# haidog-yaqub/EzAudio

Hardware: NVIDIA H100
Metric: audio-seconds generated per wall-second (EzAudio-XL, 50-step DDIM, 10 s) (higher is better)
Workload: dtype bf16

## Files before the change

### ezaudio_b200/csrc/common.cuh

```cuda
#pragma once
#include <cuda.h>
#include <cuda_bf16.h>
#include <cuda_runtime.h>
#include <stdint.h>

#include "wgmma.cuh"

namespace ezb {

__device__ __forceinline__ uint32_t smem_u32(const void* p) { return (uint32_t)__cvta_generic_to_shared(p); }

__device__ __forceinline__ bool elect_one() {
  uint32_t pred;
  asm volatile(
      "{\n\t.reg .pred p;\n\telect.sync _|p, 0xffffffff;\n\tselp.u32 %0, 1, 0, p;\n\t}\n"
      : "=r"(pred));
  return pred != 0;
}

__device__ __forceinline__ void pdl_wait() { asm volatile("griddepcontrol.wait;" ::: "memory"); }
__device__ __forceinline__ void pdl_launch() { asm volatile("griddepcontrol.launch_dependents;" ::: "memory"); }

__device__ __forceinline__ void mbar_init(uint64_t* bar, uint32_t count) {
  asm volatile("mbarrier.init.shared::cta.b64 [%0], %1;" ::"r"(smem_u32(bar)), "r"(count));
}
__device__ __forceinline__ void fence_mbar_init() { asm volatile("fence.mbarrier_init.release.cluster;" ::: "memory"); }
__device__ __forceinline__ void mbar_expect_tx(uint64_t* bar, uint32_t bytes) {
  asm volatile("mbarrier.arrive.expect_tx.shared::cta.b64 _, [%0], %1;" ::"r"(smem_u32(bar)), "r"(bytes) : "memory");
}
__device__ __forceinline__ void mbar_arrive(uint64_t* bar) {
  asm volatile("mbarrier.arrive.shared::cta.b64 _, [%0];" ::"r"(smem_u32(bar)) : "memory");
}
__device__ __forceinline__ void mbar_wait(uint64_t* bar, uint32_t parity) {
  asm volatile(
      "{\n\t.reg .pred P1;\n\t"
      "WAIT_LOOP:\n\t"
      "mbarrier.try_wait.parity.shared::cta.b64 P1, [%0], %1, 0x989680;\n\t"
      "@P1 bra DONE;\n\t"
      "bra WAIT_LOOP;\n\t"
      "DONE:\n\t}\n" ::"r"(smem_u32(bar)),
      "r"(parity)
      : "memory");
}

__device__ __forceinline__ void fence_proxy_async_smem() { asm volatile("fence.proxy.async.shared::cta;" ::: "memory"); }
__device__ __forceinline__ void named_bar_sync(int id, int nthreads) {
  asm volatile("bar.sync %0, %1;" ::"r"(id), "r"(nthreads) : "memory");
}

__device__ __forceinline__ void tma_prefetch_desc(const CUtensorMap* m) {
  asm volatile("prefetch.tensormap [%0];" ::"l"(reinterpret_cast<uint64_t>(m)) : "memory");
}
__device__ __forceinline__ void tma_load_2d(void* dst, const CUtensorMap* m, uint64_t* bar, int c0, int c1) {
  asm volatile(
      "cp.async.bulk.tensor.2d.shared::cluster.global.mbarrier::complete_tx::bytes [%0], [%1, {%3, %4}], [%2];" ::"r"(
          smem_u32(dst)),
      "l"(reinterpret_cast<uint64_t>(m)), "r"(smem_u32(bar)), "r"(c0), "r"(c1)
      : "memory");
}
__device__ __forceinline__ void tma_load_3d(void* dst, const CUtensorMap* m, uint64_t* bar, int c0, int c1, int c2) {
  asm volatile(
      "cp.async.bulk.tensor.3d.shared::cluster.global.mbarrier::complete_tx::bytes [%0], [%1, {%3, %4, %5}], [%2];" ::"r"(
          smem_u32(dst)),
      "l"(reinterpret_cast<uint64_t>(m)), "r"(smem_u32(bar)), "r"(c0), "r"(c1), "r"(c2)
      : "memory");
}

__device__ __forceinline__ void tma_load_4d(void* dst, const CUtensorMap* m, uint64_t* bar, int c0, int c1, int c2, int c3) {
  asm volatile(
      "cp.async.bulk.tensor.4d.shared::cluster.global.mbarrier::complete_tx::bytes [%0], [%1, {%3, %4, %5, %6}], [%2];" ::"r"(
          smem_u32(dst)),
      "l"(reinterpret_cast<uint64_t>(m)), "r"(smem_u32(bar)), "r"(c0), "r"(c1), "r"(c2), "r"(c3)
      : "memory");
}
__device__ __forceinline__ void tma_store_2d(const CUtensorMap* m, const void* src, int c0, int c1) {
  asm volatile("cp.async.bulk.tensor.2d.global.shared::cta.bulk_group [%0, {%2, %3}], [%1];" ::"l"(reinterpret_cast<uint64_t>(m)),
               "r"(smem_u32(src)), "r"(c0), "r"(c1)
               : "memory");
}
__device__ __forceinline__ void bulk_commit_group() { asm volatile("cp.async.bulk.commit_group;" ::: "memory"); }
template <int N>
__device__ __forceinline__ void bulk_wait_group_read() { asm volatile("cp.async.bulk.wait_group.read %0;" ::"n"(N) : "memory"); }
template <int N>
__device__ __forceinline__ void bulk_wait_group() { asm volatile("cp.async.bulk.wait_group %0;" ::"n"(N) : "memory"); }

__device__ __forceinline__ uint64_t wgmma_desc_sw128(uint32_t smem_addr) {
  uint64_t d = 0;
  d |= (uint64_t)((smem_addr & 0x3FFFF) >> 4);
  d |= (uint64_t)1 << 16;
  d |= (uint64_t)(1024 >> 4) << 32;
  d |= (uint64_t)1 << 62;
  return d;
}
__device__ __forceinline__ uint64_t wgmma_desc_sw32(uint32_t smem_addr) {
  uint64_t d = 0;
  d |= (uint64_t)((smem_addr & 0x3FFFF) >> 4);
  d |= (uint64_t)1 << 16;
  d |= (uint64_t)(256 >> 4) << 32;
  d |= (uint64_t)3 << 62;
  return d;
}
__device__ __forceinline__ void wgmma_fence() { asm volatile("wgmma.fence.sync.aligned;" ::: "memory"); }
__device__ __forceinline__ void wgmma_commit() { asm volatile("wgmma.commit_group.sync.aligned;" ::: "memory"); }
template <int N>
__device__ __forceinline__ void wgmma_wait() { asm volatile("wgmma.wait_group.sync.aligned %0;" ::"n"(N) : "memory"); }
template <int R>
__device__ __forceinline__ void wgmma_fence_regs(float (&d)[R]) {
#pragma unroll
  for (int i = 0; i < R; ++i) asm volatile("" : "+f"(d[i])::"memory");
}

__device__ __forceinline__ float gelu_erf(float x) { return 0.5f * x * (1.0f + erff(x * 0.70710678118654752440f)); }
__device__ __forceinline__ float silu(float x) { return x / (1.0f + expf(-x)); }
__device__ __forceinline__ uint32_t pack_bf16(float a, float b) {
  __nv_bfloat162 v = __floats2bfloat162_rn(a, b);
  return *reinterpret_cast<uint32_t*>(&v);
}
__device__ __forceinline__ float warp_sum(float v) {
#pragma unroll
  for (int o = 16; o > 0; o >>= 1) v += __shfl_xor_sync(0xffffffffu, v, o);
  return v;
}
__device__ __forceinline__ float warp_max(float v) {
#pragma unroll
  for (int o = 16; o > 0; o >>= 1) v = fmaxf(v, __shfl_xor_sync(0xffffffffu, v, o));
  return v;
}

}

namespace ezb {
__device__ __forceinline__ uint32_t cluster_ctarank() {
  uint32_t r;
  asm volatile("mov.u32 %0, %%cluster_ctarank;" : "=r"(r));
  return r;
}
__device__ __forceinline__ void cluster_sync_all() {
  asm volatile("barrier.cluster.arrive.release.aligned;" ::: "memory");
  asm volatile("barrier.cluster.wait.acquire.aligned;" ::: "memory");
}
__device__ __forceinline__ uint32_t mapa_u32(uint32_t local_addr, uint32_t rank) {
  uint32_t r;
  asm volatile("mapa.shared::cluster.u32 %0, %1, %2;" : "=r"(r) : "r"(local_addr), "r"(rank));
  return r;
}
__device__ __forceinline__ void mbar_arrive_cluster(uint32_t cluster_addr) {
  asm volatile("mbarrier.arrive.release.cluster.shared::cluster.b64 _, [%0];" ::"r"(cluster_addr) : "memory");
}
__device__ __forceinline__ void mbar_arrive_cluster_nofence(uint32_t cluster_addr) {
  asm volatile("mbarrier.arrive.shared::cluster.b64 _, [%0];" ::"r"(cluster_addr) : "memory");
}
__device__ __forceinline__ void mbar_inval(uint64_t* bar) {
  asm volatile("mbarrier.inval.shared::cta.b64 [%0];" ::"r"(smem_u32(bar)) : "memory");
}
__device__ __forceinline__ void tma_load_2d_mc(void* dst, const CUtensorMap* m, uint64_t* bar, int c0, int c1, uint16_t mask) {
  asm volatile(
      "cp.async.bulk.tensor.2d.shared::cluster.global.mbarrier::complete_tx::bytes.multicast::cluster [%0], [%1, {%3, %4}], [%2], %5;" ::"r"(
          smem_u32(dst)),
      "l"(reinterpret_cast<uint64_t>(m)), "r"(smem_u32(bar)), "r"(c0), "r"(c1), "h"(mask)
      : "memory");
}
}
```

### ezaudio_b200/csrc/gemm.cuh

```cuda
#pragma once
#include "common.cuh"

namespace ezb {

constexpr int GEMM_BM = 128;
constexpr int GEMM_BK = 64;
#ifdef EZB_GEMM_DEBUG
#define EZB_DBG(...) __VA_ARGS__
#else
#define EZB_DBG(...)
#endif
constexpr int GEMM_SMEM_BUDGET = 227 * 1024 - 2048;
constexpr int gemm_b_box(int bn) { return bn > 256 ? bn / 2 : bn; }

struct GemmShape {
  int M, N;
  int num_k_blocks;
  int num_m_tiles, num_n_tiles;
  int taps, center, dilation, cin_blocks, T, tiles_per_batch;
  int stride, pad;
  unsigned long long* dbg;
  const char* pf;
  unsigned int pf_bytes;
};
// ... 301 lines not shown
    const EpiLinearParams& e = ep.lin;
    const int nv = nvalid < 32 ? nvalid : 32;
    wait();
#pragma unroll 1
    for (int c = c_begin; c < c_end; c += 64) {
      const int col = n0 + c + 2 * lane;
      const bool col_ok = (c + 2 * lane < c_end) && col < N;
      __syncwarp();
#pragma unroll
      for (int hc = 0; hc < 2; ++hc) {
        uint32_t r[32];
        acc_ld<32>(ar, c + 32 * hc, lane, r);
#pragma unroll
        for (int g = 0; g < 16; ++g) stage_put(st, lane, 16 * hc + g, __uint_as_float(r[2 * g]), __uint_as_float(r[2 * g + 1]));
      }
      __syncwarp();
      if (!col_ok) continue;
      const float b0 = e.bias != nullptr ? e.bias[col] : 0.f, b1 = e.bias != nullptr ? e.bias[col + 1] : 0.f;
#pragma unroll 4
      for (int rr = 0; rr < nv; ++rr) {
        const int row = row0 + rr;
        const float s = ep.scale[row / ep.rows_per_batch];
        const float2 acc = stage_get(st, rr, lane);
        *reinterpret_cast<float2*>(e.out_f32 + (size_t)row * e.ld32 + col) = make_float2((acc.x + b0) * s, (acc.y + b1) * s);
      }
    }
  }
};

struct EpiGegluParams {
  const float* bias;
  __nv_bfloat16* out_bf16;
  int ld16;
  int split_stride;
  FoldIn fin;
};
__device__ __forceinline__ float rcp_approx(float x) {
  float r;
  asm("rcp.approx.ftz.f32 %0, %1;" : "=f"(r) : "f"(x));
  return r;
}
__device__ __forceinline__ float ex2_approx(float x) {
  float r;
  asm("ex2.approx.ftz.f32 %0, %1;" : "=f"(r) : "f"(x));
  return r;
}
__device__ __forceinline__ float geglu_fast(float h, float g) {
  const float z = g * 0.70710678118654752440f, az = fabsf(z);
  const float t = rcp_approx(fmaf(0.3275911f, az, 1.0f));
  float p = fmaf(1.061405429f, t, -1.453152027f);
  p = fmaf(p, t, 1.421413741f);
  p = fmaf(p, t, -0.284496736f);
  p = fmaf(p, t, 0.254829592f);
  const float e = ex2_approx(az * az * -1.4426950408889634f);
  const float erf_abs = fmaf(-p * t, e, 1.0f);
  const float erf_s = copysignf(erf_abs, z);
  return h * (0.5f * g) * (1.0f + erf_s);
}

template <int BN, bool FOLD = false>
struct EpiGeglu {
  using Params = EpiGegluParams;
  static constexpr int HALF = BN / 2;
  static constexpr int EPI_WARPS = BN == 256 ? 8 : 4;
  static constexpr bool WIDE_REGS = false;
  static constexpr int STAGE_FLOATS = 32 * 32;
  template <class Wait>
  static __device__ __forceinline__ void run(const Params& ep, float* st, const AccRows& ar, int row0, int nvalid, int n0, int N, int lane, int c_begin,
                                             int c_end, Wait wait) {
    constexpr bool fold = FOLD;
    float rstd = 1.f, nmr = 0.f;
    if (fold && lane < nvalid) fold_row_stats(ep.fin, row0 + lane, rstd, nmr);
    wait();
    const int f_begin = c_begin / 2, f_end = c_end / 2;
#pragma unroll 1
    for (int c = f_begin; c < f_end; c += 64) {
      if (n0 + c >= N) break;
      if (ep.split_stride > 0) {
        uint32_t h[32], g[32];
#pragma unroll 1
        for (int q4 = 0; q4 < 2; ++q4) {
          __syncwarp();
          acc_ld<32>(ar, c + q4 * 32, lane, h);
          acc_ld<32>(ar, HALF + c + q4 * 32, lane, g);
          if (lane < nvalid) {
            __nv_bfloat16* o = ep.out_bf16 + (size_t)(row0 + lane) * ep.ld16 + (n0 / 2 + c + q4 * 32);
#pragma unroll
            for (int j = 0; j < 32; j += 2) {
              const float o0 = (__uint_as_float(h[j]) + ep.bias[n0 + c + q4 * 32 + j]) * gelu_erf(__uint_as_float(g[j]) + ep.bias[n0 + HALF + c + q4 * 32 + j]);
              const float o1 = (__uint_as_float(h[j + 1]) + ep.bias[n0 + c + q4 * 32 + j + 1]) * gelu_erf(__uint_as_float(g[j + 1]) + ep.bias[n0 + HALF + c + q4 * 32 + j + 1]);
              store_bf16x2(o + j, ep.split_stride, o0, o1);
            }
          }
        }
        continue;
      }
      uint32_t pk[32];
#pragma unroll
      for (int q4 = 0; q4 < 2; ++q4) {
        uint32_t h[32], g[32];
        __syncwarp();
        acc_ld<32>(ar, c + q4 * 32, lane, h);
        acc_ld<32>(ar, HALF + c + q4 * 32, lane, g);
        if (fold) {
          const float* bh = ep.fin.v + n0 + c + q4 * 32;
          const float* bg = ep.fin.v + n0 + HALF + c + q4 * 32;
          const float* uh = ep.fin.u + n0 + c + q4 * 32;
          const float* ug = ep.fin.u + n0 + HALF + c + q4 * 32;
#pragma unroll
          for (int j = 0; j < 32; j += 2) {
            const float o0 = geglu_fast(fmaf(__uint_as_float(h[j]), rstd, fmaf(nmr, __ldg(uh + j), __ldg(bh + j))),
                                        fmaf(__uint_as_float(g[j]), rstd, fmaf(nmr, __ldg(ug + j), __ldg(bg + j))));
            const float o1 = geglu_fast(fmaf(__uint_as_float(h[j + 1]), rstd, fmaf(nmr, __ldg(uh + j + 1), __ldg(bh + j + 1))),
                                        fmaf(__uint_as_float(g[j + 1]), rstd, fmaf(nmr, __ldg(ug + j + 1), __ldg(bg + j + 1))));
            pk[q4 * 16 + j / 2] = pack_bf16(o0, o1);
          }
        } else {
        const float* bh = ep.bias + n0 + c + q4 * 32;
        const float* bg = ep.bias + n0 + HALF + c + q4 * 32;
#pragma unroll
        for (int j = 0; j < 32; j += 2) {
          const float o0 = geglu_fast(__uint_as_float(h[j]) + __ldg(bh + j), __uint_as_float(g[j]) + __ldg(bg + j));
          const float o1 = geglu_fast(__uint_as_float(h[j + 1]) + __ldg(bh + j + 1), __uint_as_float(g[j + 1]) + __ldg(bg + j + 1));
          pk[q4 * 16 + j / 2] = pack_bf16(o0, o1);
        }
        }
      }
      __syncwarp();
#pragma unroll
      for (int gq = 0; gq < 16; ++gq) stage_put<32>(st, lane, gq, __uint_as_float(pk[2 * gq]), __uint_as_float(pk[2 * gq + 1]));
      __syncwarp();
      const int hl = lane & 15, hw = lane >> 4;
      __nv_bfloat16* obase = ep.out_bf16 + (size_t)row0 * ep.ld16 + (n0 / 2 + c + 4 * hl);
#pragma unroll 4
      for (int rp = 0; rp < 16; ++rp) {
        const int rr = 2 * rp + hw;
        if (rr < nvalid) *reinterpret_cast<float2*>(obase + (size_t)rr * ep.ld16) = stage_get<32>(st, rr, hl);
      }
    }
  }
};

__device__ __forceinline__ void warpgroup_bar_sync(int wg) {
  if (wg == 0) named_bar_sync(2, 128);
  else named_bar_sync(3, 128);
}
struct EpiGegluFrag {
  using Params = EpiGegluParams;
  static constexpr bool FRAG = true;
  static constexpr int EPI_WARPS = 8;
  static constexpr bool WIDE_REGS = false;
  static constexpr int STAGE_FLOATS = 32 * 32;
  static constexpr int HALF = 128;
  static __device__ __forceinline__ void frag(const Params& ep, const CUtensorMap* out, float (&d)[128], uint8_t* tile, int m0, int n0, const GemmShape&,
                                              int wg, int lg, int lane) {
    const int q = lane & 3;
    const int r0 = 16 * lg + (lane >> 2);
    const float2* bh = reinterpret_cast<const float2*>(ep.bias + n0) + q;
    const float2* bg = reinterpret_cast<const float2*>(ep.bias + n0 + HALF) + q;
#pragma unroll
    for (int i = 0; i < 16; ++i) {
      const float2 b_h = __ldg(bh + 4 * i), b_g = __ldg(bg + 4 * i);
      const uint32_t lo = pack_bf16(geglu_fast(d[4 * i] + b_h.x, d[64 + 4 * i] + b_g.x), geglu_fast(d[4 * i + 1] + b_h.y, d[64 + 4 * i + 1] + b_g.y));
      const uint32_t hi = pack_bf16(geglu_fast(d[4 * i + 2] + b_h.x, d[64 + 4 * i + 2] + b_g.x), geglu_fast(d[4 * i + 3] + b_h.y, d[64 + 4 * i + 3] + b_g.y));
      uint8_t* p = tile + (i >> 3) * 8192 + r0 * 128 + (((i & 7) ^ (r0 & 7)) << 4) + 4 * q;
      *reinterpret_cast<uint32_t*>(p) = lo;
      *reinterpret_cast<uint32_t*>(p + 8 * 128) = hi;
    }
    fence_proxy_async_smem();
    warpgroup_bar_sync(wg);
    if ((threadIdx.x & 127) == 0) {
      tma_store_2d(out, tile, n0 / 2, m0 + 64 * wg);
      tma_store_2d(out, tile + 8192, n0 / 2 + 64, m0 + 64 * wg);
      bulk_commit_group();
    }
  }
};
template <class E>
constexpr auto epi_frag_impl(int) -> decltype(E::FRAG) { return E::FRAG; }
template <class E>
constexpr bool epi_frag_impl(long) { return false; }
template <class E>
constexpr bool epi_frag() { return epi_frag_impl<E>(0); }

__device__ __forceinline__ int swap_chunk_tokens(int c, int c_end, int t0, int N) {
  int n = c_end - c;
  if (N - t0 < n) n = N - t0;
  return n < 32 ? n : 32;
}
template <int BN>
struct EpiLinearT {
  using Params = EpiLinearParams;
  static constexpr int EPI_WARPS = 8;
  static constexpr bool WIDE_REGS = false;
  static constexpr int STAGE_FLOATS = 0;
  static __device__ __forceinline__ void load_resid(const Params& ep, float (&x)[32], int t0, int nt, int f, bool f_ok) {
#pragma unroll
    for (int j = 0; j < 32; ++j) x[j] = (f_ok && j < nt) ? ep.resid[(size_t)(t0 + j) * ep.ldr + f] : 0.f;
  }
  template <class Wait>
  static __device__ __forceinline__ void run(const Params& ep, float* st, const AccRows& ar, int row0, int nvalid, int n0, int N, int lane, int c_begin,
                                             int c_end, Wait wait) {
    const int f = row0 + lane;
    const bool f_ok = lane < nvalid;
    const float bias = (ep.bias != nullptr && f_ok) ? ep.bias[f] : 0.f;
    bool waited = false;
    float x[32];
    if (ep.resid != nullptr && n0 + c_begin < N) load_resid(ep, x, n0 + c_begin, swap_chunk_tokens(c_begin, c_end, n0 + c_begin, N), f, f_ok);
#pragma unroll 1
    for (int c = c_begin; c < c_end; c += 32) {
      const int t0 = n0 + c;
      if (t0 >= N) break;
      const int nt = swap_chunk_tokens(c, c_end, t0, N);
      float xn[32];
      const bool more = ep.resid != nullptr && c + 32 < c_end && t0 + 32 < N;
      if (more) load_resid(ep, xn, t0 + 32, swap_chunk_tokens(c + 32, c_end, t0 + 32, N), f, f_ok);
      float g0 = 1.f, g1 = 1.f;
      int btok = 0x7fffffff;
      if (ep.gate != nullptr && f_ok) {
        const int b0i = t0 / ep.rows_per_batch;
        btok = (b0i + 1) * ep.rows_per_batch;
        g0 = 1.0f - ep.gate[(size_t)b0i * ep.gate_bstride + f];
        if (btok < t0 + nt) g1 = 1.0f - ep.gate[(size_t)(b0i + 1) * ep.gate_bstride + f];
      }
      if (!waited) { wait(); waited = true; }
      uint32_t r[32];
      __syncwarp();
      acc_ld<32>(ar, c, lane, r);
      if (f_ok) {
        float* o = ep.out_f32 + (size_t)t0 * ep.ld32 + f;
#pragma unroll
        for (int j = 0; j < 32; ++j) {
          if (j >= nt) break;
          float v = __uint_as_float(r[j]) + bias;
          if (ep.resid != nullptr) v = fmaf((t0 + j >= btok) ? g1 : g0, v, x[j]);
          o[(size_t)j * ep.ld32] = v;
        }
      }
      if (more) {
#pragma unroll
        for (int j = 0; j < 32; ++j) x[j] = xn[j];
      }
    }
    if (!waited) wait();
  }
};

template <int BN>
struct EpiLinearTF {
  using Params = EpiLinearParams;
  static constexpr int EPI_WARPS = 8;
  static constexpr bool WIDE_REGS = false;
  static constexpr int STAGE_FLOATS = 0;
  template <class Wait>
  static __device__ __forceinline__ void run(const Params& ep, float* st, const AccRows& ar, int row0, int nvalid, int n0, int N, int lane, int c_begin,
                                             int c_end, Wait wait) {
    const int f = row0 + lane;
    const bool f_ok = lane < nvalid;
    const float bias = (ep.bias != nullptr && f_ok) ? ep.bias[f] : 0.f;
    const bool fold_in = ep.fin.u != nullptr, fold_out = ep.fout.st != nullptr && nvalid > 0;
    float uf = 0.f, vf = 0.f, ga = 1.f, gb = 1.f;
    if (fold_in && f_ok) { uf = ep.fin.u[f]; vf = ep.fin.v[f]; }
    if (fold_out && f_ok) {
      if (ep.fout.g0 != nullptr) ga = ep.fout.g0[f];
      if (ep.fout.a1 != nullptr && ep.fout.g1 != nullptr) gb = ep.fout.g1[f];
    }
    bool waited = false;
#pragma unroll 1
    for (int c = c_begin; c < c_end; c += 32) {
      const int t0 = n0 + c;
      if (t0 >= N) break;
      const int nt = swap_chunk_tokens(c, c_end, t0, N);
      float x[32];
      if (ep.resid != nullptr) {
#pragma unroll
        for (int j = 0; j < 32; ++j) x[j] = (f_ok && j < nt) ? ep.resid[(size_t)(t0 + j) * ep.ldr + f] : 0.f;
      }
      float g0 = 1.f, g1 = 1.f;
      int btok = 0x7fffffff;
      if (ep.gate != nullptr && f_ok) {
        const int b0i = t0 / ep.rows_per_batch;
        btok = (b0i + 1) * ep.rows_per_batch;
        g0 = 1.0f - ep.gate[(size_t)b0i * ep.gate_bstride + f];
        if (btok < t0 + nt) g1 = 1.0f - ep.gate[(size_t)(b0i + 1) * ep.gate_bstride + f];
      }
      float rs_l = 1.f, nm_l = 0.f;
      if (fold_in && lane < nt) fold_row_stats(ep.fin, t0 + lane, rs_l, nm_l);
      if (!waited) { wait(); waited = true; }
      uint32_t r[32];
      __syncwarp();
      acc_ld<32>(ar, c, lane, r);
      float val[32];
#pragma unroll
      for (int j = 0; j < 32; ++j) {
        float acc = __uint_as_float(r[j]);
        if (fold_in) {
          const float rs = __shfl_sync(0xffffffffu, rs_l, j), nm = __shfl_sync(0xffffffffu, nm_l, j);
          acc = fmaf(acc, rs, fmaf(nm, uf, vf));
        }
        float v = acc + bias;
        float gj = (t0 + j >= btok) ? g1 : g0;
        if (ep.resid != nullptr) v = fmaf(gj, v, x[j]);
        val[j] = (f_ok && j < nt) ? v : 0.f;
      }
      if (f_ok) {
        float* o = ep.out_f32 + (size_t)t0 * ep.ld32 + f;
// ... 97 lines not shown
    wgmma_commit();
    if (kb > 0) { wgmma_wait<1>(); release(prev); }
    prev = stage;
    if (++stage == SM::STAGES) { stage = 0; phase ^= 1; }
  }
  wgmma_wait<0>();
  release(prev);
#pragma unroll
  for (int s = 0; s < NSUB; ++s)
#pragma unroll
    for (int h = 0; h < NH; ++h) wgmma_fence_regs(d[s][h]);
}

template <int BN, class Epi, int MC, bool FP8 = false>
__device__ __forceinline__ void gemm_mma_part(int row64, const uint8_t* sA, const uint8_t* sB, float* sAcc, uint64_t* full, uint64_t* empty,
                                              int num_k_blocks, uint32_t& stage, uint32_t& phase, int lg, int lane, const Fp8Scales& fs = Fp8Scales{},
                                              int m0 = 0, int M = 0, int n0 = 0) {
  using SM = GemmCfg<BN, Epi>;
  constexpr int NSUB = SM::NSUB, NH = SM::NH, HN = SM::HN;
  float d[NSUB][NH][HN / 2];
  gemm_mainloop<BN, Epi, MC, FP8>(d, row64, sA, sB, full, empty, num_k_blocks, stage, phase);
  named_bar_sync(1, 32 * SM::EPI_WARPS);
  if constexpr (FP8) {
#pragma unroll
    for (int s = 0; s < NSUB; ++s) {
      const int r = m0 + (row64 + s) * 64 + 16 * lg + (lane >> 2);
      const float sa0 = r < M ? fs.sa[r] : 0.f, sa1 = r + 8 < M ? fs.sa[r + 8] : 0.f;
#pragma unroll
      for (int h = 0; h < NH; ++h) {
        const float2* sw = reinterpret_cast<const float2*>(fs.sw + n0 + h * HN + 2 * (lane & 3));
#pragma unroll
        for (int i = 0; i < HN / 8; ++i) {
          const float2 w = __ldg(sw + 4 * i);
          d[s][h][4 * i] *= sa0 * w.x; d[s][h][4 * i + 1] *= sa0 * w.y;
          d[s][h][4 * i + 2] *= sa1 * w.x; d[s][h][4 * i + 3] *= sa1 * w.y;
        }
      }
    }
  }
#pragma unroll
  for (int s = 0; s < NSUB; ++s) {
#pragma unroll
    for (int h = 0; h < NH; ++h) {
      float* r0 = sAcc + (size_t)((row64 + s) * 64 + 16 * lg + (lane >> 2)) * SM::ACC_PITCH + h * HN + 2 * (lane & 3);
#pragma unroll
      for (int i = 0; i < HN / 8; ++i) {
        *reinterpret_cast<float2*>(r0 + 8 * i) = make_float2(d[s][h][4 * i], d[s][h][4 * i + 1]);
        *reinterpret_cast<float2*>(r0 + 8 * SM::ACC_PITCH + 8 * i) = make_float2(d[s][h][4 * i + 2], d[s][h][4 * i + 3]);
      }
    }
  }
}

template <int BN>
struct McSub { static constexpr int ROWS = BN % 32 == 0 ? 32 : 16; };
template <int R>
__device__ __forceinline__ void setmaxnreg_inc() { asm volatile("setmaxnreg.inc.sync.aligned.u32 %0;" ::"n"(R)); }
template <int R>
__device__ __forceinline__ void setmaxnreg_dec() { asm volatile("setmaxnreg.dec.sync.aligned.u32 %0;" ::"n"(R)); }
template <int BN, class Epi, int MC = 1, bool FIRST_PHASE = false, bool FP8 = false>
__device__ __forceinline__ void gemm_body(const CUtensorMap& tmA, const CUtensorMap& tmB, const GemmShape& g, const typename Epi::Params& ep, uint8_t* smem_raw,
                                          const Fp8Scales& fs = Fp8Scales{}, const CUtensorMap* tmC = nullptr) {
  using SM = GemmCfg<BN, Epi>;
  constexpr int KB_ELEMS = FP8 ? 2 * GEMM_BK : GEMM_BK;
  static_assert(BN % 16 == 0 && BN >= 64 && (BN <= 256 || (BN <= 512 && BN % 32 == 0 && MC == 1 && SM::MMA_WG == 2)), "BN");
  static_assert(MC >= 1 && MC <= 8 && BN % McSub<BN>::ROWS == 0, "MC");
  constexpr int STAGES = SM::STAGES, EPI_WARPS = SM::EPI_WARPS, NSUB = SM::NSUB;
  constexpr uint16_t MC_MASK = static_cast<uint16_t>((1u << MC) - 1u);
  uint8_t* smem = smem_raw + ((1024u - (smem_u32(smem_raw) & 1023u)) & 1023u);
  uint8_t* sA = smem;
  uint8_t* sB = smem + STAGES * SM::A_BYTES;
  float* sAcc = reinterpret_cast<float*>(smem);
  float* sStage = reinterpret_cast<float*>(smem + SM::RING);
  uint64_t* full = reinterpret_cast<uint64_t*>(smem + SM::RING + SM::STAGE_BYTES);
  uint64_t* empty = full + STAGES;
  uint64_t* acc_free = empty + STAGES;

  const int warp = threadIdx.x >> 5;
  const int lane = threadIdx.x & 31;
  const int num_tiles = g.num_m_tiles * g.num_n_tiles;
  constexpr int PRODUCER = EPI_WARPS;

  if (warp == PRODUCER && lane == 0) {
    tma_prefetch_desc(&tmA);
    tma_prefetch_desc(&tmB);
    for (int i = 0; i < STAGES; ++i) {
      mbar_init(&full[i], 1);
      mbar_init(&empty[i], SM::MMA_WG * MC);
    }
    mbar_init(acc_free, EPI_WARPS * MC);
    fence_mbar_init();
  }
  __syncthreads();
  if (MC > 1) cluster_sync_all();
  pdl_launch();
  if (warp == PRODUCER && g.pf_bytes != 0) {
    if (elect_one()) prefetch_weights_l2(g.pf, g.pf_bytes, blockIdx.x, gridDim.x);
    __syncwarp();
  }
  pdl_wait();
  EZB_DBG(const bool dbg = g.dbg != nullptr && blockIdx.x == 0; const long long t_start = clock64(); long long w0 = 0, w1 = 0, w4 = 0;)

  if (warp >= PRODUCER) {
    if constexpr (SM::PRODUCER_WG) setmaxnreg_dec<SM::REGS_PRODUCER>();
    uint32_t stage = 0, phase = 0, af_phase = 0;
    bool first = true;
    for (int tile = warp == PRODUCER ? (int)blockIdx.x : num_tiles; tile < num_tiles; tile += gridDim.x) {
      const int mt = tile % g.num_m_tiles, nt = tile / g.num_m_tiles;
      const int n0 = nt * BN;
      if (!SM::FRAG && !first) { mbar_wait(acc_free, af_phase); af_phase ^= 1; }
      first = false;
      for (int kb = 0; kb < g.num_k_blocks; ++kb) {
        EZB_DBG(const long long tq = clock64();)
        mbar_wait(&empty[stage], phase ^ 1);
        EZB_DBG(w0 += clock64() - tq;)
        if (elect_one()) {
          mbar_expect_tx(&full[stage], SM::A_BYTES + SM::B_BYTES);
          uint8_t* dA = sA + stage * SM::A_BYTES;
          uint8_t* dB = sB + stage * SM::B_BYTES;
          if (g.taps == 0) {
            tma_load_2d(dA, &tmA, &full[stage], kb * KB_ELEMS, mt * GEMM_BM);
          } else {
            const int tap = kb / g.cin_blocks, cb = kb - tap * g.cin_blocks;
            const int bidx = mt / g.tiles_per_batch, t0 = (mt - bidx * g.tiles_per_batch) * GEMM_BM;
            if (g.stride > 1) {
              const int off = tap - g.pad;
              const int r = ((off % g.stride) + g.stride) % g.stride, dq = (off - r) / g.stride;
              tma_load_4d(dA, &tmA, &full[stage], cb * GEMM_BK, r, t0 + dq, bidx);
            } else {
              tma_load_3d(dA, &tmA, &full[stage], cb * GEMM_BK, t0 + (tap - g.center) * g.dilation, bidx);
            }
          }
          if (MC == 1) {
            constexpr int BOX = gemm_b_box(BN);
#pragma unroll
            for (int j = 0; j < BN / BOX; ++j) tma_load_2d(dB + j * BOX * 128, &tmB, &full[stage], kb * KB_ELEMS, n0 + j * BOX);
          } else {
            constexpr int SR = McSub<BN>::ROWS;
            for (int j = (int)cluster_ctarank(); j < BN / SR; j += MC)
              tma_load_2d_mc(dB + j * SR * 128, &tmB, &full[stage], kb * KB_ELEMS, n0 + j * SR, MC_MASK);
          }
        }
        __syncwarp();
        if (++stage == STAGES) { stage = 0; phase ^= 1; }
      }
    }
  } else {
    if constexpr (SM::PRODUCER_WG) setmaxnreg_inc<SM::REGS_CONSUMER>();
    const int wg = warp >> 2, lg = warp & 3;
    uint32_t stage = 0, phase = 0;
    if constexpr (SM::FRAG) {
      static_assert(!FP8 && !FIRST_PHASE, "FRAG: bf16 kernels of one phase (gemm_frag_kernel)");
      uint8_t* tile_buf = reinterpret_cast<uint8_t*>(sStage) + wg * (SM::STAGE_BYTES / 2);
      for (int tile = blockIdx.x; tile < num_tiles; tile += gridDim.x) {
        const int mt = tile % g.num_m_tiles, nt = tile / g.num_m_tiles;
        EZB_DBG(const long long tm = clock64();)
        float d[NSUB][SM::NH][SM::HN / 2] = {};
        gemm_mainloop<BN, Epi, MC>(d, wg * NSUB, sA, sB, full, empty, g.num_k_blocks, stage, phase);
        EZB_DBG(const long long ta = clock64(); w0 += ta - tm;)
        if ((threadIdx.x & 127) == 0) bulk_wait_group_read<0>();
        warpgroup_bar_sync(wg);
        EZB_DBG(const long long te = clock64(); w1 += te - ta;)
        Epi::frag(ep, tmC, d[0][0], tile_buf, mt * GEMM_BM, nt * BN, g, wg, lg, lane);
        EZB_DBG(w4 += clock64() - te;)
      }
      if ((threadIdx.x & 127) == 0) bulk_wait_group<0>();
    } else
    for (int tile = blockIdx.x; tile < num_tiles; tile += gridDim.x) {
      const int mt = tile % g.num_m_tiles, nt = tile / g.num_m_tiles;
      EZB_DBG(const long long tm = clock64();)
      gemm_mma_part<BN, Epi, MC, FP8>(wg * NSUB, sA, sB, sAcc, full, empty, g.num_k_blocks, stage, phase, lg, lane, fs, mt * GEMM_BM, g.M, nt * BN);
      EZB_DBG(const long long ta = clock64(); w0 += ta - tm;)
      named_bar_sync(1, 32 * EPI_WARPS);
      EZB_DBG(const long long te = clock64(); w1 += te - ta;)
      int row0, nvalid;
      if (g.taps == 0) {
        row0 = mt * GEMM_BM + lg * 32;
        nvalid = g.M - row0;
      } else {
        const int bidx = mt / g.tiles_per_batch, t0 = (mt - bidx * g.tiles_per_batch) * GEMM_BM + lg * 32;
        row0 = bidx * g.T + t0;
        nvalid = g.T - t0;
      }
      constexpr int CW = BN / (EPI_WARPS / 4);
      const AccRows ar{sAcc + lg * 32 * SM::ACC_PITCH, SM::ACC_PITCH};
      Epi::run(ep, sStage + warp * Epi::STAGE_FLOATS, ar, row0, nvalid, nt * BN, g.N, lane, wg * CW, (wg + 1) * CW, []() {});
      EZB_DBG(w4 += clock64() - te;)
      fence_proxy_async_smem();
      __syncwarp();
      if (lane == 0) {
        if (MC == 1) mbar_arrive(acc_free);
        else for (int r = 0; r < MC; ++r) mbar_arrive_cluster(mapa_u32(smem_u32(acc_free), r));
      }
    }
    if constexpr (SM::PRODUCER_WG) setmaxnreg_dec<SM::REGS_LAUNCH>();
  }
  EZB_DBG(if (dbg && lane == 0) {
    if (warp == PRODUCER) atomicAdd(&g.dbg[2], (unsigned long long)w0);
    if (warp == 0) {
      atomicAdd(&g.dbg[0], (unsigned long long)w0); atomicAdd(&g.dbg[1], (unsigned long long)w1); atomicAdd(&g.dbg[4], (unsigned long long)w4);
      atomicAdd(&g.dbg[5], (unsigned long long)(clock64() - t_start));
    }
  })
  __syncthreads();
  if constexpr (SM::PRODUCER_WG) if (warp >= PRODUCER) setmaxnreg_inc<SM::REGS_LAUNCH>();
  if (MC > 1) cluster_sync_all();
  if (FIRST_PHASE) {
    if (warp == PRODUCER && lane == 0) {
      for (int i = 0; i < STAGES; ++i) { mbar_inval(&full[i]); mbar_inval(&empty[i]); }
      mbar_inval(acc_free);
    }
    __syncthreads();
  }
}
template <int BN, class Epi, int MC = 1>
__global__ void __launch_bounds__((GemmCfg<BN, Epi>::THREADS), 1)
gemm_wgmma_kernel(const __grid_constant__ CUtensorMap tmA, const __grid_constant__ CUtensorMap tmB, const GemmShape g,
                  const typename Epi::Params ep) {
  extern __shared__ uint8_t smem_dyn[];
  gemm_body<BN, Epi, MC>(tmA, tmB, g, ep, smem_dyn);
}
template <int BN, class Epi>
__global__ void __launch_bounds__((GemmCfg<BN, Epi>::THREADS), 1)
gemm_frag_kernel(const __grid_constant__ CUtensorMap tmA, const __grid_constant__ CUtensorMap tmB, const __grid_constant__ CUtensorMap tmC,
                 const GemmShape g, const typename Epi::Params ep) {
  extern __shared__ uint8_t smem_dyn[];
  gemm_body<BN, Epi, 2>(tmA, tmB, g, ep, smem_dyn, Fp8Scales{}, &tmC);
}
template <int BN, class Epi>
__global__ void __launch_bounds__((GemmCfg<BN, Epi>::THREADS), 1)
gemm_fp8_kernel(const __grid_constant__ CUtensorMap tmA, const __grid_constant__ CUtensorMap tmB, const GemmShape g, const typename Epi::Params ep,
                const Fp8Scales fs) {
  extern __shared__ uint8_t smem_dyn[];
  gemm_body<BN, Epi, 2, false, true>(tmA, tmB, g, ep, smem_dyn, fs);
}

}

namespace ezb {
struct EpiHeadsParams {
  int D, H, L;
  int kind[3];
  float nw[2][72];
  float nb[2][72];
  const float2* rope;
  int rope_ld;
  int rope_mufu;
  float inv_freq[36];
  int rope_kinds;
  __nv_bfloat16* out[3];
  int ld_qk, dvp, Lpad;
  int dbg;
  FoldIn fin;
};

constexpr int heads_bn(int dh, int hpt) { return hpt == 3 ? (dh == 72 ? 224 : 3 * dh) : 2 * dh; }
template <int DH, int HPT>
__device__ __forceinline__ bool head_of_tile(const EpiHeadsParams& ep, int n0, int hh, int N, int& sec, int& head) {
  if (HPT == 3) {
    const int g = (n0 / heads_bn(DH, HPT)) * 3 + hh;
    sec = g / ep.H;
    head = g - sec * ep.H;
    return true;
  }
  const int n = n0 + hh * DH;
  if (n >= N) return false;
  sec = n / ep.D;
  head = (n - sec * ep.D) / DH;
  return true;
}
template <int DH, bool DBG>
__device__ __forceinline__ void head_ln_rope(const EpiHeadsParams& ep, float (&v)[DH], int kind, int l) {
  float s1[4] = {0.f, 0.f, 0.f, 0.f}, s2[4] = {0.f, 0.f, 0.f, 0.f};
#pragma unroll
  for (int i = 0; i < DH; ++i) { s1[i & 3] += v[i]; s2[i & 3] = fmaf(v[i], v[i], s2[i & 3]); }
  const float mean = ((s1[0] + s1[1]) + (s1[2] + s1[3])) * (1.0f / DH);
  const float var = fmaxf(((s2[0] + s2[1]) + (s2[2] + s2[3])) * (1.0f / DH) - mean * mean, 0.f);
  const float rstd = rsqrtf(var + 1e-5f);
  const float nmr = -mean * rstd;
  if (DBG && (ep.dbg & 2)) {
  } else if (kind == 0) {
#pragma unroll
    for (int i = 0; i < DH; ++i) v[i] = fmaf(fmaf(v[i], rstd, nmr), ep.nw[0][i], ep.nb[0][i]);
  } else {
#pragma unroll
    for (int i = 0; i < DH; ++i) v[i] = fmaf(fmaf(v[i], rstd, nmr), ep.nw[1][i], ep.nb[1][i]);
  }
  if (ep.rope != nullptr && ((ep.rope_kinds >> kind) & 1) && !(DBG && (ep.dbg & 1))) {
    const float2* cs = ep.rope + (size_t)l * (DH / 2);
    const float lf = (float)l;
#pragma unroll
    for (int i = 0; i < DH / 2; ++i) {
      float2 c;
      if (ep.rope_mufu) __sincosf(lf * ep.inv_freq[i], &c.y, &c.x);
      else c = __ldg(cs + i);
      const float a = v[i], bq = v[i + DH / 2];
      v[i] = a * c.x - bq * c.y;
      v[i + DH / 2] = bq * c.x + a * c.y;
    }
  }
}
template <int DH>
__device__ __forceinline__ void head_store_row(const EpiHeadsParams& ep, const float (&v)[DH], int kind, size_t bh, int l) {
  uint4* dst = reinterpret_cast<uint4*>(ep.out[kind] + (bh * ep.L + l) * (size_t)ep.ld_qk);
#pragma unroll
  for (int g = 0; g < DH / 8; ++g)
    dst[g] = make_uint4(pack_bf16(v[8 * g], v[8 * g + 1]), pack_bf16(v[8 * g + 2], v[8 * g + 3]), pack_bf16(v[8 * g + 4], v[8 * g + 5]),
                        pack_bf16(v[8 * g + 6], v[8 * g + 7]));
}
template <int DH>
__device__ __forceinline__ void head_store_vt(const EpiHeadsParams& ep, const float (&v)[DH], size_t bh, int l) {
  __nv_bfloat16* dst = ep.out[2] + bh * ep.dvp * ep.Lpad + l;
#pragma unroll
  for (int i = 0; i < DH; ++i) { *dst = __float2bfloat16_rn(v[i]); dst += ep.Lpad; }
  for (int i = DH; i < ep.dvp; ++i) { *dst = __float2bfloat16_rn(0.f); dst += ep.Lpad; }
}

template <int DH, int HPT = 2, bool FOLD = false, bool DBG = false>
struct EpiHeads {
  using Params = EpiHeadsParams;
  static constexpr int BN = heads_bn(DH, HPT);
  static constexpr int EPI_WARPS = 8;
  static constexpr bool WIDE_REGS = HPT == 3;
  static constexpr int STAGE_FLOATS = EPI_STAGE_FLOATS;
  template <class Wait>
  static __device__ __forceinline__ void run(const Params& ep, float* st, const AccRows& ar, int row0, int nvalid, int n0, int N, int lane, int c_begin,
                                             int c_end, Wait wait) {
    const int row = row0 + lane;
    const bool row_ok = lane < nvalid;
    constexpr bool fold = FOLD;
    float f_rstd = 1.f, f_nmr = 0.f;
    if (fold && row_ok) fold_row_stats(ep.fin, row, f_rstd, f_nmr);
    wait();
    const int b = row_ok ? row / ep.L : 0, l = row_ok ? row - b * ep.L : 0;
#pragma unroll 1
    for (int hh = threadIdx.x >> 7; hh < HPT; hh += 2) {
      int sec, head;
      if (!head_of_tile<DH, HPT>(ep, n0, hh, N, sec, head)) break;
      const int kind = ep.kind[sec];
      uint32_t r[DH];
      __syncwarp();
      acc_ld<64>(ar, hh * DH, lane, r);
      if constexpr (DH == 72) acc_ld<8>(ar, hh * DH + 64, lane, r + 64);
      float v[DH];
#pragma unroll
      for (int i = 0; i < DH; ++i) v[i] = __uint_as_float(r[i]);
      if (fold) {
        const float4* u4 = reinterpret_cast<const float4*>(ep.fin.u + n0 + hh * DH);
        const float4* v4 = reinterpret_cast<const float4*>(ep.fin.v + n0 + hh * DH);
#pragma unroll
        for (int i = 0; i < DH / 4; ++i) {
          const float4 uu = __ldg(u4 + i), vv = __ldg(v4 + i);
          v[4 * i] = fmaf(v[4 * i], f_rstd, fmaf(f_nmr, uu.x, vv.x));
          v[4 * i + 1] = fmaf(v[4 * i + 1], f_rstd, fmaf(f_nmr, uu.y, vv.y));
          v[4 * i + 2] = fmaf(v[4 * i + 2], f_rstd, fmaf(f_nmr, uu.z, vv.z));
          v[4 * i + 3] = fmaf(v[4 * i + 3], f_rstd, fmaf(f_nmr, uu.w, vv.w));
        }
      }
      const size_t bh = (size_t)b * ep.H + head;
      if (kind < 2) {
        head_ln_rope<DH, DBG>(ep, v, kind, l);
#pragma unroll
        for (int g = 0; g < DH / 4; ++g)
          stage_put(st, lane, g, __uint_as_float(pack_bf16(v[4 * g], v[4 * g + 1])), __uint_as_float(pack_bf16(v[4 * g + 2], v[4 * g + 3])));
        __syncwarp();
        if (lane < DH / 4 && !(DBG && (ep.dbg & 8))) {
          const int rb0 = row0 / ep.L, rl0 = row0 - rb0 * ep.L;
          __nv_bfloat16* base = ep.out[kind] + 4 * lane;
          const size_t head_rows = (size_t)ep.L * ep.ld_qk;
          const int nv = nvalid < 32 ? nvalid : 32;
#pragma unroll 4
          for (int rr = 0; rr < nv; ++rr) {
            int rl = rl0 + rr, rb = rb0;
            while (rl >= ep.L) { rl -= ep.L; ++rb; }
            *reinterpret_cast<float2*>(base + ((size_t)rb * ep.H + head) * head_rows + (size_t)rl * ep.ld_qk) = stage_get(st, rr, lane);
          }
        }
      } else if (row_ok && !(DBG && (ep.dbg & 4))) {
        head_store_vt<DH>(ep, v, bh, l);
      }
    }
  }
};

template <int DH, int HPT>
struct EpiHeadsFrag {
  using Params = EpiHeadsParams;
  static constexpr bool FRAG = true;
  static constexpr int BN = heads_bn(DH, HPT);
  static constexpr int EPI_WARPS = 8;
  static constexpr bool WIDE_REGS = true;
  static constexpr int PITCH = DH + 4;
  static constexpr int STAGE_FLOATS = 64 * PITCH / 4;
  static_assert(DH % 8 == 0, "head slices start on a fragment register quad");
  static __device__ __forceinline__ void frag(const Params& ep, const CUtensorMap*, float (&d)[BN / 2], uint8_t* tile, int m0, int n0, const GemmShape& g,
                                              int wg, int lg, int lane) {
    float* buf = reinterpret_cast<float*>(tile);
    const int t = threadIdx.x & 127, half = t >> 6;
    const int row = m0 + 64 * wg + (t & 63);
    const bool row_ok = row < g.M;
    const int b = row_ok ? row / ep.L : 0, l = row_ok ? row - b * ep.L : 0;
    float* w0 = buf + (16 * lg + (lane >> 2)) * PITCH + 2 * (lane & 3);
    const float4* rd = reinterpret_cast<const float4*>(buf + (t & 63) * PITCH);
#pragma unroll
    for (int p = 0; p < HPT; p += 2) {
      float v[DH];
#pragma unroll
      for (int s = 0; s < 2; ++s) {
        const int hh = p + s;
        if (hh >= HPT) break;
        if (hh > 0) warpgroup_bar_sync(wg);
#pragma unroll
        for (int i = 0; i < DH / 8; ++i) {
          const int j = 4 * (hh * DH / 8 + i);
          *reinterpret_cast<float2*>(w0 + 8 * i) = make_float2(d[j], d[j + 1]);
          *reinterpret_cast<float2*>(w0 + 8 * PITCH + 8 * i) = make_float2(d[j + 2], d[j + 3]);
        }
        warpgroup_bar_sync(wg);
        if (half == s) {
#pragma unroll
          for (int i = 0; i < DH / 4; ++i) {
            const float4 x = rd[i];
            v[4 * i] = x.x; v[4 * i + 1] = x.y; v[4 * i + 2] = x.z; v[4 * i + 3] = x.w;
          }
        }
      }
      const int hh = p + half;
      int sec, head;
      if (hh >= HPT || !head_of_tile<DH, HPT>(ep, n0, hh, g.N, sec, head)) continue;
      const int kind = ep.kind[sec];
      const size_t bh = (size_t)b * ep.H + head;
      if (kind < 2) {
        head_ln_rope<DH, false>(ep, v, kind, l);
        if (row_ok) head_store_row<DH>(ep, v, kind, bh, l);
      } else if (row_ok) {
        head_store_vt<DH>(ep, v, bh, l);
      }
    }
  }
};

}

namespace ezb {
struct GridBarrier { unsigned int count; unsigned int gen; };
__device__ __forceinline__ void grid_barrier(GridBarrier* b) {
  __syncthreads();
  if (threadIdx.x == 0) {
    __threadfence();
    unsigned int gen;
    asm volatile("ld.acquire.gpu.global.u32 %0, [%1];" : "=r"(gen) : "l"(&b->gen) : "memory");
    if (atomicAdd(&b->count, 1u) == gridDim.x - 1) {
      b->count = 0;
      __threadfence();
      asm volatile("st.release.gpu.global.u32 [%0], %1;" ::"l"(&b->gen), "r"(gen + 1) : "memory");
    } else {
      unsigned int cur;
      do {
        asm volatile("ld.acquire.gpu.global.u32 %0, [%1];" : "=r"(cur) : "l"(&b->gen) : "memory");
      } while (cur == gen);
    }
  }
  __syncthreads();
  asm volatile("fence.proxy.async;" ::: "memory");
}
template <int BN1, class Epi1, class Epi2>
__global__ void __launch_bounds__((GemmCfg<BN1, Epi1>::THREADS), 1)
mlp_fused_kernel(const __grid_constant__ CUtensorMap tmA1, const __grid_constant__ CUtensorMap tmB1, const GemmShape g1, const typename Epi1::Params ep1,
                 const __grid_constant__ CUtensorMap tmA2, const __grid_constant__ CUtensorMap tmB2, const GemmShape g2, const typename Epi2::Params ep2,
                 GridBarrier* bar) {
  static_assert(GemmCfg<BN1, Epi1>::THREADS == GemmCfg<256, Epi2>::THREADS, "both phases use the same warp roles");
  extern __shared__ uint8_t smem_dyn[];
  gemm_body<BN1, Epi1, 2, true>(tmA1, tmB1, g1, ep1, smem_dyn);
  grid_barrier(bar);
  gemm_body<256, Epi2, 1>(tmA2, tmB2, g2, ep2, smem_dyn);
}

}
```

Before: 51.37.

## Apply per-head LayerNorm and RoPE on fragments and stage outputs via stmatrix

Reworks the fused QKV-heads GEMM epilogue. LayerNorm statistics and RoPE are now computed directly on the wgmma accumulator fragments using warp shuffles, with LN weights and RoPE frequencies cached once in shared memory. Results are packed to bf16 and staged with stmatrix (transposed for V) into double-buffered swizzled slots, then written to global memory as coalesced 16-byte stores. This drops the fp32 shared-memory round trip and the per-thread row gathers, at the cost of more complex indexing, unaligned-store fallbacks for V, and some added register pressure.

```diff
diff --git a/ezaudio_b200/csrc/common.cuh b/ezaudio_b200/csrc/common.cuh
--- a/ezaudio_b200/csrc/common.cuh
+++ b/ezaudio_b200/csrc/common.cuh
@@ -77,6 +77,18 @@
   asm volatile("cp.async.bulk.tensor.2d.global.shared::cta.bulk_group [%0, {%2, %3}], [%1];" ::"l"(reinterpret_cast<uint64_t>(m)),
                "r"(smem_u32(src)), "r"(c0), "r"(c1)
                : "memory");
+}
+__device__ __forceinline__ void stmatrix_x4(void* p, uint32_t r0, uint32_t r1, uint32_t r2, uint32_t r3) {
+  asm volatile("stmatrix.sync.aligned.m8n8.x4.shared.b16 [%0], {%1, %2, %3, %4};" ::"r"(smem_u32(p)), "r"(r0), "r"(r1), "r"(r2), "r"(r3) : "memory");
+}
+__device__ __forceinline__ void stmatrix_x2(void* p, uint32_t r0, uint32_t r1) {
+  asm volatile("stmatrix.sync.aligned.m8n8.x2.shared.b16 [%0], {%1, %2};" ::"r"(smem_u32(p)), "r"(r0), "r"(r1) : "memory");
+}
+__device__ __forceinline__ void stmatrix_x4_trans(void* p, uint32_t r0, uint32_t r1, uint32_t r2, uint32_t r3) {
+  asm volatile("stmatrix.sync.aligned.m8n8.x4.trans.shared.b16 [%0], {%1, %2, %3, %4};" ::"r"(smem_u32(p)), "r"(r0), "r"(r1), "r"(r2), "r"(r3) : "memory");
+}
+__device__ __forceinline__ void stmatrix_x2_trans(void* p, uint32_t r0, uint32_t r1) {
+  asm volatile("stmatrix.sync.aligned.m8n8.x2.trans.shared.b16 [%0], {%1, %2};" ::"r"(smem_u32(p)), "r"(r0), "r"(r1) : "memory");
 }
 __device__ __forceinline__ void bulk_commit_group() { asm volatile("cp.async.bulk.commit_group;" ::: "memory"); }
 template <int N>
diff --git a/ezaudio_b200/csrc/gemm.cuh b/ezaudio_b200/csrc/gemm.cuh
--- a/ezaudio_b200/csrc/gemm.cuh
+++ b/ezaudio_b200/csrc/gemm.cuh
@@ -477,6 +477,7 @@
   static constexpr bool WIDE_REGS = false;
   static constexpr int STAGE_FLOATS = 32 * 32;
   static constexpr int HALF = 128;
+  static __device__ __forceinline__ void setup(const Params&, uint8_t*) {}
   static __device__ __forceinline__ void frag(const Params& ep, const CUtensorMap* out, float (&d)[128], uint8_t* tile, int m0, int n0, const GemmShape&,
                                               int wg, int lg, int lane) {
     const int q = lane & 3;
@@ -880,6 +881,7 @@
     if constexpr (SM::FRAG) {
       static_assert(!FP8 && !FIRST_PHASE, "FRAG: bf16 kernels of one phase (gemm_frag_kernel)");
       uint8_t* tile_buf = reinterpret_cast<uint8_t*>(sStage) + wg * (SM::STAGE_BYTES / 2);
+      Epi::setup(ep, tile_buf);
       for (int tile = blockIdx.x; tile < num_tiles; tile += gridDim.x) {
         const int mt = tile % g.num_m_tiles, nt = tile / g.num_m_tiles;
         EZB_DBG(const long long tm = clock64();)
@@ -1027,14 +1029,6 @@
       v[i + DH / 2] = bq * c.x + a * c.y;
     }
   }
-}
-template <int DH>
-__device__ __forceinline__ void head_store_row(const EpiHeadsParams& ep, const float (&v)[DH], int kind, size_t bh, int l) {
-  uint4* dst = reinterpret_cast<uint4*>(ep.out[kind] + (bh * ep.L + l) * (size_t)ep.ld_qk);
-#pragma unroll
-  for (int g = 0; g < DH / 8; ++g)
-    dst[g] = make_uint4(pack_bf16(v[8 * g], v[8 * g + 1]), pack_bf16(v[8 * g + 2], v[8 * g + 3]), pack_bf16(v[8 * g + 4], v[8 * g + 5]),
-                        pack_bf16(v[8 * g + 6], v[8 * g + 7]));
 }
 template <int DH>
 __device__ __forceinline__ void head_store_vt(const EpiHeadsParams& ep, const float (&v)[DH], size_t bh, int l) {
@@ -1118,52 +1112,195 @@
   static constexpr int BN = heads_bn(DH, HPT);
   static constexpr int EPI_WARPS = 8;
   static constexpr bool WIDE_REGS = true;
-  static constexpr int PITCH = DH + 4;
-  static constexpr int STAGE_FLOATS = 64 * PITCH / 4;
-  static_assert(DH % 8 == 0, "head slices start on a fragment register quad");
-  static __device__ __forceinline__ void frag(const Params& ep, const CUtensorMap*, float (&d)[BN / 2], uint8_t* tile, int m0, int n0, const GemmShape& g,
+  static constexpr int QK_PITCH = DH == 64 ? 128 : 2 * DH;
+  static constexpr int SLOT = DH * 128;
+  static constexpr int TABLE = 2048;
+  static constexpr int STAGE_FLOATS = 2 * (2 * SLOT + TABLE) / (4 * EPI_WARPS);
+  static_assert(DH % 8 == 0 && 5 * DH * 4 <= TABLE && (2 * SLOT + TABLE) % 1024 == 0, "heads staging");
+
+  static __device__ __forceinline__ void setup(const Params& ep, uint8_t* buf) {
+    float* tab = reinterpret_cast<float*>(buf + 2 * SLOT);
+    const int i = threadIdx.x & 127;
+    if (i < DH) {
+      tab[i] = ep.nw[0][i]; tab[DH + i] = ep.nb[0][i]; tab[2 * DH + i] = ep.nw[1][i]; tab[3 * DH + i] = ep.nb[1][i];
+      tab[4 * DH + i] = ep.inv_freq[i % (DH / 2)];
+    }
+  }
+
+  static __device__ __forceinline__ void ln_rope(const Params& ep, float* x, int kind, const float* tab, int q, const float (&lf)[2], const int (&lp)[2]) {
+    const bool lo = (q & 2) == 0;
+    float s1[2][2] = {{0.f, 0.f}, {0.f, 0.f}}, s2[2][2] = {{0.f, 0.f}, {0.f, 0.f}};
+#pragma unroll
+    for (int g = 0; g < DH / 8; ++g) {
+#pragma unroll
+      for (int k = 0; k < 4; ++k) {
+        const float own = x[4 * g + k], oth = __shfl_xor_sync(0xffffffffu, own, 2);
+        const float f = lo ? own : oth, s = lo ? oth : own;
+        float& a = s1[k >> 1][k & 1];
+        float& b = s2[k >> 1][k & 1];
+        a += f; b = fmaf(f, f, b);
+        a += s; b = fmaf(s, s, b);
+      }
+    }
+    float rstd[2], nmr[2];
+#pragma unroll
+    for (int h = 0; h < 2; ++h) {
+      const float p1 = s1[h][0] + s1[h][1], p2 = s2[h][0] + s2[h][1];
+      const float t1 = p1 + __shfl_xor_sync(0xffffffffu, p1, 1), t2 = p2 + __shfl_xor_sync(0xffffffffu, p2, 1);
+      const float mean = t1 * (1.0f / DH);
+      const float var = fmaxf(__fmaf_rn(t2, 1.0f / DH, -__fmul_rn(mean, mean)), 0.f);
+      rstd[h] = rsqrtf(var + 1e-5f);
+      nmr[h] = -mean * rstd[h];
+    }
+    const float2* w = reinterpret_cast<const float2*>(tab + 2 * kind * DH) + q;
+    const float2* bb = reinterpret_cast<const float2*>(tab + (2 * kind + 1) * DH) + q;
+#pragma unroll
+    for (int g = 0; g < DH / 8; ++g) {
+      const float2 wv = w[4 * g], bv = bb[4 * g];
+      x[4 * g] = fmaf(fmaf(x[4 * g], rstd[0], nmr[0]), wv.x, bv.x);
+      x[4 * g + 1] = fmaf(fmaf(x[4 * g + 1], rstd[0], nmr[0]), wv.y, bv.y);
+      x[4 * g + 2] = fmaf(fmaf(x[4 * g + 2], rstd[1], nmr[1]), wv.x, bv.x);
+      x[4 * g + 3] = fmaf(fmaf(x[4 * g + 3], rstd[1], nmr[1]), wv.y, bv.y);
+    }
+    if (ep.rope == nullptr || !((ep.rope_kinds >> kind) & 1)) return;
+    constexpr int NG = DH / 8;
+    float y[DH / 2];
+#pragma unroll
+    for (int g = 0; g < NG; ++g) {
+#pragma unroll
+      for (int k = 0; k < 4; ++k) {
+        if constexpr (DH == 72) y[4 * g + k] = __shfl_xor_sync(0xffffffffu, lo ? x[4 * ((g + 5) % NG) + k] : x[4 * ((g + 4) % NG) + k], 2);
+        else y[4 * g + k] = x[4 * ((g + 4) % NG) + k];
+      }
+    }
+    const float2* fr = reinterpret_cast<const float2*>(tab + 4 * DH) + q;
+#pragma unroll
+    for (int g = 0; g < NG; ++g) {
+      const float2 f2 = fr[4 * g];
+      const bool first = g < 4 || (DH == 72 && g == 4 && lo);
+#pragma unroll
+      for (int k = 0; k < 4; ++k) {
+        const int h = k >> 1;
+        float2 c;
+        if (ep.rope_mufu) __sincosf(lf[h] * ((k & 1) ? f2.y : f2.x), &c.y, &c.x);
+        else c = __ldg(ep.rope + (size_t)lp[h] * (DH / 2) + (8 * g + 2 * q + (k & 1)) % (DH / 2));
+        const float own = x[4 * g + k], oth = y[4 * g + k];
+        x[4 * g + k] = first ? __fmaf_rn(own, c.x, -__fmul_rn(oth, c.y)) : __fmaf_rn(oth, c.y, __fmul_rn(own, c.x));
+      }
+    }
+  }
+
+  static __device__ __forceinline__ void stage(const float* x, int kind, uint8_t* slot, int lg, int lane) {
+    const int mi = lane >> 3, ri = lane & 7;
+    if (kind < 2) {
+      const int row = 16 * lg + 8 * (mi & 1) + ri;
+#pragma unroll
+      for (int g = 0; g < DH / 8; g += 2) {
+        const int chunk = g + (mi >> 1);
+        uint8_t* p = slot + row * QK_PITCH + 16 * (DH == 64 ? (chunk ^ (row & 7)) : chunk);
+        if (g + 1 < DH / 8)
+          stmatrix_x4(p, pack_bf16(x[4 * g], x[4 * g + 1]), pack_bf16(x[4 * g + 2], x[4 * g + 3]), pack_bf16(x[4 * g + 4], x[4 * g + 5]),
+                      pack_bf16(x[4 * g + 6], x[4 * g + 7]));
+        else
+          stmatrix_x2(p, pack_bf16(x[4 * g], x[4 * g + 1]), pack_bf16(x[4 * g + 2], x[4 * g + 3]));
+      }
+    } else {
+      const int chunk = 2 * lg + (mi & 1);
+#pragma unroll
+      for (int g = 0; g < DH / 8; g += 2) {
+        const int d = 8 * (g + (mi >> 1)) + ri;
+        uint8_t* p = slot + d * 128 + 16 * (chunk ^ ri);
+        if (g + 1 < DH / 8)
+          stmatrix_x4_trans(p, pack_bf16(x[4 * g], x[4 * g + 1]), pack_bf16(x[4 * g + 2], x[4 * g + 3]), pack_bf16(x[4 * g + 4], x[4 * g + 5]),
+                            pack_bf16(x[4 * g + 6], x[4 * g + 7]));
+        else
+          stmatrix_x2_trans(p, pack_bf16(x[4 * g], x[4 * g + 1]), pack_bf16(x[4 * g + 2], x[4 * g + 3]));
+      }
+    }
+  }
+
+  static __device__ __forceinline__ void clip_of(const Params& ep, int b0, int l0, int r, int& b, int& l) {
+    b = b0;
+    l = l0 + r;
+    while (l >= ep.L) { l -= ep.L; ++b; }
+  }
+  static __device__ __forceinline__ void write(const Params& ep, const uint8_t* slot, int kind, int head, int rs, int b0, int l0, int M, int t) {
+    if (kind < 2) {
+      constexpr int CH = DH / 8;
+#pragma unroll 1
+      for (int c = t; c < 64 * CH; c += 128) {
+        const int r = c / CH, k = c - r * CH;
+        if (rs + r >= M) break;
+        int b, l;
+        clip_of(ep, b0, l0, r, b, l);
+        const uint4 v = *reinterpret_cast<const uint4*>(slot + r * QK_PITCH + 16 * (DH == 64 ? (k ^ (r & 7)) : k));
+        *reinterpret_cast<uint4*>(ep.out[kind] + (((size_t)b * ep.H + head) * ep.L + l) * ep.ld_qk + 8 * k) = v;
+      }
+      return;
+    }
+#pragma unroll 1
+    for (int c = t; c < ep.dvp * 8; c += 128) {
+      const int d = c >> 3, k = c & 7;
+      if (rs + 8 * k >= M) continue;
+      uint4 v = make_uint4(0u, 0u, 0u, 0u);
+      if (d < DH) v = *reinterpret_cast<const uint4*>(slot + d * 128 + 16 * (k ^ (d & 7)));
+      int b, l;
+      clip_of(ep, b0, l0, 8 * k, b, l);
+      __nv_bfloat16* dst = ep.out[2] + (((size_t)b * ep.H + head) * ep.dvp + d) * ep.Lpad + l;
+      const uintptr_t a = reinterpret_cast<uintptr_t>(dst);
+      if (l + 8 <= ep.L && rs + 8 * k + 8 <= M) {
+        if ((a & 15) == 0) {
+          *reinterpret_cast<uint4*>(dst) = v;
+        } else if ((a & 7) == 0) {
+          reinterpret_cast<uint2*>(dst)[0] = make_uint2(v.x, v.y);
+          reinterpret_cast<uint2*>(dst)[1] = make_uint2(v.z, v.w);
+        } else if ((a & 3) == 0) {
+          uint32_t* o = reinterpret_cast<uint32_t*>(dst);
+          o[0] = v.x; o[1] = v.y; o[2] = v.z; o[3] = v.w;
+        } else {
+          const uint32_t w[4] = {v.x, v.y, v.z, v.w};
+          unsigned short* o = reinterpret_cast<unsigned short*>(dst);
+#pragma unroll
+          for (int j = 0; j < 8; ++j) o[j] = (unsigned short)(w[j >> 1] >> (16 * (j & 1)));
+        }
+      } else {
+        const uint32_t w[4] = {v.x, v.y, v.z, v.w};
+#pragma unroll
+        for (int j = 0; j < 8; ++j) {
+          if (rs + 8 * k + j >= M) break;
+          int bj, lj;
+          clip_of(ep, b0, l0, 8 * k + j, bj, lj);
+          *reinterpret_cast<unsigned short*>(ep.out[2] + (((size_t)bj * ep.H + head) * ep.dvp + d) * ep.Lpad + lj) = (unsigned short)(w[j >> 1] >> (16 * (j & 1)));
+        }
+      }
+    }
+  }
+
+  static __device__ __forceinline__ void frag(const Params& ep, const CUtensorMap*, float (&d)[BN / 2], uint8_t* buf, int m0, int n0, const GemmShape& g,
                                               int wg, int lg, int lane) {
-    float* buf = reinterpret_cast<float*>(tile);
-    const int t = threadIdx.x & 127, half = t >> 6;
-    const int row = m0 + 64 * wg + (t & 63);
-    const bool row_ok = row < g.M;
-    const int b = row_ok ? row / ep.L : 0, l = row_ok ? row - b * ep.L : 0;
-    float* w0 = buf + (16 * lg + (lane >> 2)) * PITCH + 2 * (lane & 3);
-    const float4* rd = reinterpret_cast<const float4*>(buf + (t & 63) * PITCH);
-#pragma unroll
-    for (int p = 0; p < HPT; p += 2) {
-      float v[DH];
-#pragma unroll
-      for (int s = 0; s < 2; ++s) {
-        const int hh = p + s;
-        if (hh >= HPT) break;
-        if (hh > 0) warpgroup_bar_sync(wg);
-#pragma unroll
-        for (int i = 0; i < DH / 8; ++i) {
-          const int j = 4 * (hh * DH / 8 + i);
-          *reinterpret_cast<float2*>(w0 + 8 * i) = make_float2(d[j], d[j + 1]);
-          *reinterpret_cast<float2*>(w0 + 8 * PITCH + 8 * i) = make_float2(d[j + 2], d[j + 3]);
-        }
-        warpgroup_bar_sync(wg);
-        if (half == s) {
-#pragma unroll
-          for (int i = 0; i < DH / 4; ++i) {
-            const float4 x = rd[i];
-            v[4 * i] = x.x; v[4 * i + 1] = x.y; v[4 * i + 2] = x.z; v[4 * i + 3] = x.w;
-          }
-        }
-      }
-      const int hh = p + half;
+    const int t = threadIdx.x & 127, q = lane & 3;
+    const float* tab = reinterpret_cast<const float*>(buf + 2 * SLOT);
+    const int rs = m0 + 64 * wg;
+    const int b0 = rs / ep.L, l0 = rs - b0 * ep.L;
+    float lf[2];
+    int lp[2];
+#pragma unroll
+    for (int h = 0; h < 2; ++h) {
+      const int row = rs + 16 * lg + (lane >> 2) + 8 * h;
+      lp[h] = row - (row / ep.L) * ep.L;
+      lf[h] = (float)lp[h];
+    }
+#pragma unroll
+    for (int hh = 0; hh < HPT; ++hh) {
       int sec, head;
-      if (hh >= HPT || !head_of_tile<DH, HPT>(ep, n0, hh, g.N, sec, head)) continue;
+      head_of_tile<DH, HPT>(ep, n0, hh, g.N, sec, head);
       const int kind = ep.kind[sec];
-      const size_t bh = (size_t)b * ep.H + head;
-      if (kind < 2) {
-        head_ln_rope<DH, false>(ep, v, kind, l);
-        if (row_ok) head_store_row<DH>(ep, v, kind, bh, l);
-      } else if (row_ok) {
-        head_store_vt<DH>(ep, v, bh, l);
-      }
+      float* x = d + hh * (DH / 2);
+      if (kind < 2) ln_rope(ep, x, kind, tab, q, lf, lp);
+      uint8_t* slot = buf + (hh & 1) * SLOT;
+      stage(x, kind, slot, lg, lane);
+      warpgroup_bar_sync(wg);
+      write(ep, slot, kind, head, rs, b0, l0, g.M, t);
     }
   }
 };
```

After: 51.54 (median of 6 runs). About the same (+0.3%).
